# llsurreal919/Reduce-Complexity-for-intra-coding-of-VVC

Hardware: NVIDIA B200
Metric: all-intra 1080p10 CTUs/sec (exhaustive RMD sweep: intra pred + SAD/SATD + mode cost + candidate lists) (higher is better)
Workload: dtype int16 samples / int32 arithmetic / f64 costs

## Files before the change

vvc_intra_b200/csrc/vvcb_api.cu:

```cuda
#include <cuda_runtime.h>
#include <stdio.h>
#include <string.h>
#include <stdlib.h>
#include <math.h>
#include <new>
#include "vvcb_rmd.cuh"
#include "vvcb_tu.cuh"
#include "vvcb_feat.cuh"
#include "vvcb_dq.cuh"
#include "vvcb_rate.cuh"
#include "vvcb_chroma.cuh"
#include <vector>
#include <algorithm>
#include <time.h>
#include <thread>
#include <atomic>
#include "vvcb_romfill.h"

template <int KIND>
__global__ void __launch_bounds__(256) int_peak_kernel(const int* in, int* out, int iters)
{
  int a[8], b[8];
  const int k0 = in[threadIdx.x & 31], k1 = in[32 + (threadIdx.x & 31)];
#pragma unroll
// ... 6 lines not shown
        if (KIND == 0)      { a[i] = a[i] * k1 + k0; b[i] = b[i] * k0 + k1; }
        else if (KIND == 1) { a[i] = (a[i] + k1) ^ k0; b[i] = (b[i] ^ k1) + k0; }
        else                { a[i] = a[i] * k1 + k0; b[i] = (b[i] + k1) ^ k0; }
      }
    }
  }
  int s = 0;
#pragma unroll
  for (int i = 0; i < 8; i++) s += a[i] ^ b[i];
  out[blockIdx.x * blockDim.x + threadIdx.x] = s;
}

constexpr int kSideStreams = 7;
enum Slot {
  kTuIn, kTuOut,
  kTuResi, kTuCoeff,
  kDqCoeff, kDqTabs, kDqScratch, kDqLists,
  kStageIn, kStageOut,
  kOrig, kReco,
  kVisits, kResults, kDetails,
  kBrief,
  kSadSatd,
  kItems,
  kPred,
  kRects, kRectSamples,
  kFeatIn, kFeatOut,
  kChroma,
  kChromaIo,
  kPinTuIn, kPinTuOut, kPinStageIn, kPinStageOut,
  kSlots
};
struct Scratch { void* p; size_t cap; bool pinned; };
struct vvcb_ctx {
  int device, bd, ctu;
  cudaStream_t stream;
  cudaEvent_t ev0, ev1;
  Rom* dRom;
  TrRom* dTrRom;
  Scratch mem[kSlots];
  DqRom* dDqRom;
  RateRom* dRateRom;
  int depQuant;
  float tuMs[4]; int tuTimed; cudaEvent_t tev[5];
  cudaStream_t sIn, sOut; cudaEvent_t evIn[2], evComp[2], evOut[2];
  cudaStream_t sKind[kSideStreams]; cudaEvent_t evPlan, evKind[kSideStreams];
  int evalStreams;
  vvcb_rmd_visit* dVisP[2]; vvcb_rmd_result* dResP[2]; bool pipeReady;
  int trusted;
  const int16_t* bOrig; const int16_t* bReco;
  int width, height, stride;
  PlanState* dPlan;
  int numSms;
  int16_t* wReco;
  int yieldSync; cudaEvent_t evYield;
  void* remote;
  uint64_t launches;
  uint64_t cuNs[8], cuCalls, tuWaitFrom;
  cudaEvent_t cev[4]; bool cuSpan;
  int timing; int timedLaunches; float kms[3]; cudaEvent_t kev[4];
  int cw, ch, cstride;
  char err[512];
};

static char g_createErr[512] = "";

#define CK(call)                                                                                          \
  do {                                                                                                    \
    cudaError_t e_ = (call);                                                                              \
// ... 77 lines not shown
  memset(ctx, 0, sizeof(*ctx));
  ctx->device = device; ctx->bd = bit_depth; ctx->ctu = ctu_size; ctx->depQuant = 1;
  for (int s = kPinTuIn; s < kSlots; s++) ctx->mem[s].pinned = true;
  auto fail = [&](const char* what, cudaError_t err) {
    snprintf(g_createErr, sizeof(g_createErr), "vvcb_create: %s: %s", what, cudaGetErrorString(err));
    vvcb_destroy(ctx);
    return VVCB_ERR_CUDA;
  };
  if ((e = cudaSetDevice(device)) != cudaSuccess) return fail("cudaSetDevice", e);
  cudaDeviceProp prop;
  if ((e = cudaGetDeviceProperties(&prop, device)) != cudaSuccess) return fail("cudaGetDeviceProperties", e);
  ctx->numSms = prop.multiProcessorCount;
  if ((e = cudaStreamCreateWithFlags(&ctx->stream, cudaStreamNonBlocking)) != cudaSuccess) return fail("cudaStreamCreate", e);
  {
    const char* env = getenv("VVCB_EVAL_STREAMS");
    const int v = env ? atoi(env) : 0;
    ctx->evalStreams = v >= 1 && v <= kSideStreams + 1 ? v : kSideStreams + 1;
  }
  for (int i = 0; i < kSideStreams; i++) {
    if ((e = cudaStreamCreateWithFlags(&ctx->sKind[i], cudaStreamNonBlocking)) != cudaSuccess) return fail("cudaStreamCreate", e);
    if ((e = cudaEventCreateWithFlags(&ctx->evKind[i], cudaEventDisableTiming)) != cudaSuccess) return fail("cudaEventCreate", e);
  }
  if ((e = cudaEventCreateWithFlags(&ctx->evPlan, cudaEventDisableTiming)) != cudaSuccess) return fail("cudaEventCreate", e);
  if ((e = cudaEventCreate(&ctx->ev0)) != cudaSuccess) return fail("cudaEventCreate", e);
  if ((e = cudaEventCreateWithFlags(&ctx->evYield, cudaEventBlockingSync | cudaEventDisableTiming)) != cudaSuccess) return fail("cudaEventCreate", e);
  if ((e = cudaEventCreate(&ctx->ev1)) != cudaSuccess) return fail("cudaEventCreate", e);
  for (int i = 0; i < 4; i++) if ((e = cudaEventCreate(&ctx->kev[i])) != cudaSuccess) return fail("cudaEventCreate", e);
  for (int i = 0; i < 4; i++) if ((e = cudaEventCreate(&ctx->cev[i])) != cudaSuccess) return fail("cudaEventCreate", e);
  for (int i = 0; i < 5; i++) if ((e = cudaEventCreate(&ctx->tev[i])) != cudaSuccess) return fail("cudaEventCreate", e);
  Rom* h = new Rom();
  fill_rom(*h);
  if ((e = cudaMalloc(&ctx->dRom, sizeof(Rom))) != cudaSuccess) { delete h; return fail("cudaMalloc(rom)", e); }
  e = cudaMemcpy(ctx->dRom, h, sizeof(Rom), cudaMemcpyHostToDevice);
  delete h;
  if (e != cudaSuccess) return fail("cudaMemcpy(rom)", e);
  if ((e = cudaMalloc(&ctx->dPlan, sizeof(PlanState))) != cudaSuccess) return fail("cudaMalloc(plan)", e);
  {
    TrRom* t = new TrRom();
    fill_tr_rom(*t);
    if ((e = cudaMalloc(&ctx->dTrRom, sizeof(TrRom))) != cudaSuccess) { delete t; return fail("cudaMalloc(trrom)", e); }
    e = cudaMemcpy(ctx->dTrRom, t, sizeof(TrRom), cudaMemcpyHostToDevice);
    delete t;
    if (e != cudaSuccess) return fail("cudaMemcpy(trrom)", e);
  }
  {
    DqRom* t = new DqRom();
// ... 12 lines not shown
  *out = ctx;
  return VVCB_OK;
}

extern "C" void vvcb_destroy(vvcb_ctx* ctx)
{
  if (!ctx) return;
  if (ctx->remote) { vvcbc_disconnect(ctx->remote); delete ctx; return; }
  cudaSetDevice(ctx->device);
  cudaStreamSynchronize(ctx->stream);
  for (Scratch& b : ctx->mem) release(b);
  cudaFree(ctx->dRom); cudaFree(ctx->dPlan); cudaFree(ctx->dTrRom); cudaFree(ctx->dRateRom); cudaFree(ctx->dDqRom);
  if (ctx->pipeReady) {
    cudaStreamSynchronize(ctx->sIn); cudaStreamSynchronize(ctx->sOut);
    for (int i = 0; i < 2; i++) { cudaFree(ctx->dVisP[i]); cudaFree(ctx->dResP[i]); cudaEventDestroy(ctx->evIn[i]); cudaEventDestroy(ctx->evComp[i]); cudaEventDestroy(ctx->evOut[i]); }
    cudaStreamDestroy(ctx->sIn); cudaStreamDestroy(ctx->sOut);
  }
  cudaEventDestroy(ctx->ev0); cudaEventDestroy(ctx->ev1); cudaEventDestroy(ctx->evYield);
  for (int i = 0; i < 4; i++) cudaEventDestroy(ctx->kev[i]);
  for (int i = 0; i < 4; i++) cudaEventDestroy(ctx->cev[i]);
  for (int i = 0; i < 5; i++) cudaEventDestroy(ctx->tev[i]);
  for (int i = 0; i < kSideStreams; i++) { cudaStreamSynchronize(ctx->sKind[i]); cudaStreamDestroy(ctx->sKind[i]); cudaEventDestroy(ctx->evKind[i]); }
  cudaEventDestroy(ctx->evPlan);
  cudaStreamDestroy(ctx->stream);
  delete ctx;
}

extern "C" int vvcb_set_option(vvcb_ctx* ctx, int option, int value)
{
  if (!ctx) return VVCB_ERR_ARG;
  if (option == VVCB_OPT_DEP_QUANT && (value == 0 || value == 1)) {
    ctx->depQuant = value;
    return ctx->remote ? vvcbc_set_option(ctx->remote, option, value, ctx->err, sizeof(ctx->err)) : VVCB_OK;
  }
  if (option == VVCB_OPT_YIELD_SYNC && value >= 0 && value <= 1000) { ctx->yieldSync = value; return VVCB_OK; }
  if (option == VVCB_OPT_TRUSTED_VISITS && (value == 0 || value == 1)) { ctx->trusted = value; return VVCB_OK; }
  snprintf(ctx->err, sizeof(ctx->err), "vvcb_set_option: unknown option %d or bad value %d", option, value);
  return VVCB_ERR_ARG;
}

static int own_planes(vvcb_ctx* ctx, int width, int height)
{
  const int pitch = (width + 63) & ~63;
  const size_t bytes = (size_t)pitch * height * sizeof(int16_t);
  int rc;
  if ((rc = grow(ctx, kOrig, bytes)) || (rc = grow(ctx, kReco, bytes))) return rc;
// ... 187 lines not shown
  }
  ctx->bOrig = static_cast<const int16_t*>(d_orig); ctx->bReco = static_cast<const int16_t*>(d_reco); ctx->wReco = nullptr;
  ctx->width = width; ctx->height = height; ctx->stride = stride;
  return VVCB_OK;
}

extern "C" int vvcb_kernel_timing(vvcb_ctx* ctx, int on)
{
  if (!ctx) return VVCB_ERR_ARG;
  ctx->timing = on; ctx->timedLaunches = 0; ctx->kms[0] = ctx->kms[1] = ctx->kms[2] = 0.f;
  ctx->tuTimed = 0; ctx->tuMs[0] = ctx->tuMs[1] = ctx->tuMs[2] = ctx->tuMs[3] = 0.f;
  return VVCB_OK;
}

extern "C" int vvcb_kernel_times(vvcb_ctx* ctx, float ms[3], int* launches)
{
  if (!ctx || !ms) return VVCB_ERR_ARG;
  for (int i = 0; i < 3; i++) ms[i] = ctx->kms[i];
  if (launches) *launches = ctx->timedLaunches;
  ctx->timedLaunches = 0; ctx->kms[0] = ctx->kms[1] = ctx->kms[2] = 0.f;
  return VVCB_OK;
}

template <int TILE, int KIND, int MODE> static void launch_eval_bucket(const EvalParams& P, int numSms, long long maxWarps, cudaStream_t stream)
{
  using Cfg = EvalCfg<MODE == 1>;
  long long grid = (long long)numSms * Cfg::kMinCtas;
  const long long maxCtas = (maxWarps + Cfg::kWarps - 1) / Cfg::kWarps;
  if (grid > maxCtas) grid = maxCtas;
  if (grid < 1) grid = 1;
  rmd_eval_kernel<TILE, KIND, MODE><<<(int)grid, Cfg::kThreads, 0, stream>>>(P);
}

static int launch_rmd(vvcb_ctx* ctx, const vvcb_rmd_visit* dVisits, int n, vvcb_rmd_result* dResults, vvcb_rmd_detail* dDetails,
                      int16_t* dPred, const vvcb_rmd_visit* hostVisits = nullptr, vvcb_rmd_brief* dBrief = nullptr)
{
  if (!ctx->bOrig) { snprintf(ctx->err, sizeof(ctx->err), "vvcb_rmd_eval: vvcb_frame_begin has not been called"); return VVCB_ERR_STATE; }
  if (n == 0) return VVCB_OK;
  static_assert(kItemTasks >= 128, "the item bound below assumes at least 128 lane-tasks per plain work item");
  int rc;
  if ((rc = grow(ctx, kItems, ((size_t)n * 60 + 8) * sizeof(WorkItem))) || (rc = grow(ctx, kSadSatd, (size_t)n * 2 * VVCB_NUM_SLOTS * sizeof(uint32_t)))) return rc;
  WorkItem* dItems = buf<WorkItem>(ctx, kItems);
  uint32_t* dScratch = buf<uint32_t>(ctx, kSadSatd);
  const bool smallPlan = hostVisits && n <= 4096;
  if (!smallPlan) CK(cudaMemsetAsync(ctx->dPlan, 0, sizeof(PlanState), ctx->stream));
  const bool tm = ctx->timing != 0;
  if (tm) CK(cudaEventRecord(ctx->kev[0], ctx->stream));
  const int pack = dPred ? 0 : 1;
  bool needAll = !hostVisits || n > 4096, need[2][kNumBuckets] = {};
  int inBucket[2][kNumBuckets] = {};
  if (!needAll)
    for (int i = 0; i < n; i++) {
      const vvcb_rmd_visit& v = hostVisits[i];
      const Shape sh = make_shape(v.log2w, v.log2h);
      const int packed = pack && small_shape_index(sh.lw, sh.lh) >= 0 ? 1 : 0;
      const bool mip = !(v.flags & VVCB_VISIT_NO_MIP) && mip_num_modes(sh.w, sh.h) > 0;
      need[packed][sh.tile * kNumKinds + KIND_ANG] = need[packed][sh.tile * kNumKinds + KIND_PDC] = true;
      inBucket[packed][sh.tile * kNumKinds + KIND_ANG]++; inBucket[packed][sh.tile * kNumKinds + KIND_PDC]++;
      if (mip) { need[packed][sh.tile * kNumKinds + KIND_MIP] = true; inBucket[packed][sh.tile * kNumKinds + KIND_MIP]++; }
    }
  int evalLaunches = 0;
  if (smallPlan) rmd_plan_small<<<1, 256, 0, ctx->stream>>>(dVisits, n, ctx->ctu, ctx->dPlan, dItems, pack);
  else {
    rmd_plan_count<<<(n + 255) / 256, 256, 0, ctx->stream>>>(dVisits, n, ctx->ctu, ctx->dPlan, pack);
    rmd_plan_scan<<<1, 32, 0, ctx->stream>>>(ctx->dPlan);
    rmd_plan_fill<<<(n + 255) / 256, 256, 0, ctx->stream>>>(dVisits, n, ctx->ctu, ctx->dPlan, dItems, pack);
  }
  if (tm) CK(cudaEventRecord(ctx->kev[1], ctx->stream));
  EvalParams P;
  P.visits = dVisits; P.items = dItems; P.plan = ctx->dPlan;
  P.sadSM = dScratch; P.satdSM = (dDetails || dPred) ? dScratch + (size_t)VVCB_NUM_SLOTS * n : nullptr; P.nVisits = n;
  P.orig = ctx->bOrig; P.reco = ctx->bReco; P.stride = ctx->stride; P.bd = ctx->bd; P.ctu = ctx->ctu; P.rom = ctx->dRom;
  P.predOut = dPred;
  const long long maxWarps = (long long)n * 8;
  static const int kindOrder[kNumKinds] = { KIND_ANG, KIND_MIP, KIND_PDC };
  static const int tileOrder[kNumClasses] = { 3, 4, 5, 1, 2, 0 };
  if (!needAll && !dPred) {
    for (int mode = 1; mode >= 0; mode--) {
      EvalAny A;
      A.n = 0;
      int cta = 0;
      const int warpsPerCta = mode ? EvalCfg<true>::kWarps : EvalCfg<false>::kWarps, minCtas = mode ? EvalCfg<true>::kMinCtas : EvalCfg<false>::kMinCtas;
      for (int ki = 0; ki < kNumKinds; ki++)
        for (int ti = 0; ti < kNumClasses; ti++) {
          const int b = tileOrder[ti] * kNumKinds + kindOrder[ki];
          if (!need[mode][b] || (mode == 0 && b < kNumKinds)) continue;
          int ctas = (inBucket[mode][b] * 8 + warpsPerCta - 1) / warpsPerCta;
          if (ctas > ctx->numSms * minCtas) ctas = ctx->numSms * minCtas;
          A.bucket[A.n] = (unsigned char)b; A.firstCta[A.n] = cta; cta += ctas; A.n++;
        }
      A.firstCta[A.n] = cta;
      if (!A.n) continue;
      if (mode) rmd_eval_any_kernel<1><<<cta, EvalCfg<true>::kThreads, 0, ctx->stream>>>(P, A);
      else      rmd_eval_any_kernel<0><<<cta, EvalCfg<false>::kThreads, 0, ctx->stream>>>(P, A);
      evalLaunches++;
    }
  } else {
  const int useStreams = needAll ? ctx->evalStreams : (ctx->evalStreams < 3 ? ctx->evalStreams : 3);
  const int nSide = useStreams - 1;
  CK(cudaEventRecord(ctx->evPlan, ctx->stream));
  for (int i = 0; i < nSide; i++) CK(cudaStreamWaitEvent(ctx->sKind[i], ctx->evPlan, 0));
  int dealt = 0;
  auto next_stream = [&]() { const int k = dealt++ % useStreams; return k == 0 ? ctx->stream : ctx->sKind[k - 1]; };
  for (int ki = 0; ki < kNumKinds; ki++)
    for (int ti = 0; ti < kNumClasses; ti++) {
      const int b = tileOrder[ti] * kNumKinds + kindOrder[ki];
      if (dPred) { if (needAll || need[0][b]) { VVCB_FOR_BUCKET(b, 2, launch_eval_bucket, P, ctx->numSms, maxWarps, next_stream()); evalLaunches++; } continue; }
      if (needAll || need[1][b]) { VVCB_FOR_BUCKET(b, 1, launch_eval_bucket, P, ctx->numSms, maxWarps, next_stream()); evalLaunches++; }
      if (b >= kNumKinds && (needAll || need[0][b])) { VVCB_FOR_BUCKET(b, 0, launch_eval_bucket, P, ctx->numSms, maxWarps, next_stream()); evalLaunches++; }
    }
  for (int i = 0; i < nSide; i++) { CK(cudaEventRecord(ctx->evKind[i], ctx->sKind[i])); CK(cudaStreamWaitEvent(ctx->stream, ctx->evKind[i], 0)); }
  }
  if (tm) CK(cudaEventRecord(ctx->kev[2], ctx->stream));
  if (dDetails) { rmd_detail_kernel<<<(n + 31) / 32, 256, 0, ctx->stream>>>(dVisits, n, ctx->ctu, dDetails, P.sadSM, P.satdSM); ctx->launches++; }
  rmd_lists_kernel<<<(n + kListThreads - 1) / kListThreads, kListThreads, 0, ctx->stream>>>(dVisits, n, ctx->ctu, dResults, dDetails, P.sadSM, P.satdSM, dBrief);
  ctx->launches += (smallPlan ? 1 : 3) + evalLaunches + 1;
  CK(cudaGetLastError());
  if (tm) {
    CK(cudaEventRecord(ctx->kev[3], ctx->stream));
    CK(cudaEventSynchronize(ctx->kev[3]));
    for (int i = 0; i < 3; i++) { float ms = 0; CK(cudaEventElapsedTime(&ms, ctx->kev[i], ctx->kev[i + 1])); ctx->kms[i] += ms; }
    ctx->timedLaunches++;
  }
  return VVCB_OK;
}

static bool qp_ok(const vvcb_ctx* ctx, int per, int rem) { return rem >= 0 && rem < 6 && per >= 0 && 6 * per + rem <= 63 + 6 * (ctx->bd - 8); }
static bool lambda_ok(double l) { return l > 0.0 && isfinite(l); }

template <class F> static int first_bad_index(int n, F ok)
{
  const int kMinPerThread = 32768;
  static int maxThreads = 0;
// ... 1594 lines not shown
```

vvc_intra_b200/csrc/vvcb_rmd.cuh:

```cuda
#pragma once
#include "vvcb_core.cuh"

using namespace vvcb;

namespace {

#ifndef VVCB_EVAL_WARPS
#define VVCB_EVAL_WARPS 8
#endif
constexpr int kWarpsPerCta = VVCB_EVAL_WARPS;
constexpr int kThreads     = kWarpsPerCta * 32;
constexpr int KIND_ANG = 0, KIND_PDC = 1, KIND_MIP = 2;

template <int LMAX> struct VisitSmem {
  int16_t lines[kNumSets][2][LMAX];
  int16_t mipBnd[8];
  int16_t mipIn[2][8];
  int     mipAux[4];
  int     pad;
};
using WarpSmem = VisitSmem<kLineMax>;

#ifndef VVCB_PACK_VISITS
#define VVCB_PACK_VISITS 8
#endif
constexpr int kPackVisits  = VVCB_PACK_VISITS;
constexpr int kLineSmall   = 52;
constexpr int kSmallShapes = 8;
constexpr int kNumBucketsAll = kNumBuckets + kSmallShapes * kNumKinds;
static_assert((sizeof(VisitSmem<kLineSmall>) / 4) % 2 == 1, "bank stride of the packed line sets");

__host__ __device__ __forceinline__ int small_shape_index(int lw, int lh)
{
  if (lw + lh > 7 || lw > 4 || lh > 4) return -1;
  if (lw == 2 && lh == 2) return 0;
  if (lw == 3 && lh == 2) return 1;
  if (lw == 2 && lh == 3) return 2;
  if (lw == 3 && lh == 3) return 3;
  if (lw == 4 && lh == 2) return 4;
  if (lw == 2 && lh == 4) return 5;
  if (lw == 4 && lh == 3) return 6;
  return 7;
}

struct PlanState {
  unsigned count[kNumBucketsAll];
  unsigned offset[kNumBucketsAll];
  unsigned fill[kNumBucketsAll];
  unsigned cursor[kNumBucketsAll];
};

#ifndef VVCB_SCRATCH_VISIT_MAJOR
#define VVCB_SCRATCH_VISIT_MAJOR 1
#endif
__host__ __device__ __forceinline__ size_t scratch_at(int slot, unsigned visit, int nVisits)
{
#if VVCB_SCRATCH_VISIT_MAJOR
  (void)nVisits;
  return (size_t)visit * VVCB_NUM_SLOTS + (size_t)slot;
#else
  return (size_t)slot * (size_t)nVisits + visit;
#endif
}

struct EvalParams {
  const vvcb_rmd_visit* visits;
  const WorkItem*       items;
  PlanState*            plan;
  uint32_t*             sadSM;
  uint32_t*             satdSM;
  int                   nVisits;
  const int16_t*        orig;
  const int16_t*        reco;
  int                   stride;
  int                   bd, ctu;
  const Rom*            rom;
  int16_t*              predOut;
};

__device__ __forceinline__ bool visit_mrl_allowed(const vvcb_rmd_visit& v, int ctu)
{
  return !(v.flags & VVCB_VISIT_NO_MRL) && (v.y & (ctu - 1)) != 0;
}

__device__ __forceinline__ int visit_num_mip(const vvcb_rmd_visit& v)
{
  return (v.flags & VVCB_VISIT_NO_MIP) ? 0 : mip_num_modes(1 << v.log2w, 1 << v.log2h);
}

__device__ __forceinline__ int mpm_dc_pos(const vvcb_rmd_visit& v)
{
  int pos = 0;
#pragma unroll
  for (int i = 5; i >= 1; i--) if (v.mpm[i] == 1) pos = i;
  return pos;
}

__device__ __forceinline__ int kind_slot_count(const vvcb_rmd_visit& v, int kind, int ctu)
{
  const bool mrl = visit_mrl_allowed(v, ctu);
// ... 13 lines not shown
  }
  if (idx < 65) return rom.angOrder[v.log2w - 2][v.log2h - 2][idx];
  const int per = 5 - (dc ? 1 : 0);
  const int j = idx - 65;
  const int li = j >= per ? 1 : 0;
  int i = 1 + (j - li * per);
  if (dc && i >= dc) i++;
  return (li ? VVCB_SLOT_MRL3 : VVCB_SLOT_MRL1) + i - 1;
}

__device__ __forceinline__ int items_of(int nSlots, int lanes, int& perItem, bool packed)
{
  if (packed) { perItem = nSlots; return nSlots ? 1 : 0; }
  perItem = lanes >= kItemTasks ? 1 : kItemTasks / lanes;
  return (nSlots + perItem - 1) / perItem;
}

__device__ __forceinline__ int bucket_of(const Shape& sh, int kind, bool packed)
{
  const int small = packed ? small_shape_index(sh.lw, sh.lh) : -1;
  return small >= 0 ? kNumBuckets + small * kNumKinds + kind : sh.tile * kNumKinds + kind;
}

__global__ void rmd_plan_count(const vvcb_rmd_visit* visits, int n, int ctu, PlanState* plan, int pack)
{
  __shared__ unsigned hist[kNumBucketsAll];
  if (threadIdx.x < kNumBucketsAll) hist[threadIdx.x] = 0;
  __syncthreads();
  const int i = blockIdx.x * blockDim.x + threadIdx.x;
  if (i < n) {
    const vvcb_rmd_visit v = visits[i];
    const Shape sh = make_shape(v.log2w, v.log2h);
    const bool packed = pack && small_shape_index(sh.lw, sh.lh) >= 0;
    for (int kind = 0; kind < kNumKinds; kind++) {
      int perItem;
      const int nItems = items_of(kind_slot_count(v, kind, ctu), sh.lanes, perItem, packed);
      if (nItems) atomicAdd(&hist[bucket_of(sh, kind, packed)], (unsigned)nItems);
    }
  }
  __syncthreads();
  if (threadIdx.x < kNumBucketsAll && hist[threadIdx.x]) atomicAdd(&plan->count[threadIdx.x], hist[threadIdx.x]);
}

__global__ void rmd_plan_scan(PlanState* plan)
{
  if (blockIdx.x == 0 && threadIdx.x == 0) {
    unsigned acc = 0;
    for (int b = 0; b < kNumBucketsAll; b++) { plan->offset[b] = acc; acc += plan->count[b]; plan->fill[b] = 0; plan->cursor[b] = 0; }
  }
}

__global__ void rmd_plan_fill(const vvcb_rmd_visit* visits, int n, int ctu, PlanState* plan, WorkItem* items, int pack)
{
  __shared__ unsigned hist[kNumBucketsAll], base[kNumBucketsAll];
  if (threadIdx.x < kNumBucketsAll) hist[threadIdx.x] = 0;
  __syncthreads();
  const int i = blockIdx.x * blockDim.x + threadIdx.x;
  vvcb_rmd_visit v;
  Shape sh = make_shape(2, 2);
  unsigned local[kNumKinds] = { 0, 0, 0 };
  int nItems[kNumKinds] = { 0, 0, 0 }, perItem[kNumKinds] = { 1, 1, 1 }, nSlots[kNumKinds] = { 0, 0, 0 };
  bool packed = false;
  if (i < n) {
    v = visits[i];
    sh = make_shape(v.log2w, v.log2h);
    packed = pack && small_shape_index(sh.lw, sh.lh) >= 0;
    for (int kind = 0; kind < kNumKinds; kind++) {
      nSlots[kind] = kind_slot_count(v, kind, ctu);
      nItems[kind] = items_of(nSlots[kind], sh.lanes, perItem[kind], packed);
      if (nItems[kind]) local[kind] = atomicAdd(&hist[bucket_of(sh, kind, packed)], (unsigned)nItems[kind]);
    }
  }
  __syncthreads();
  if (threadIdx.x < kNumBucketsAll && hist[threadIdx.x])
    base[threadIdx.x] = plan->offset[threadIdx.x] + atomicAdd(&plan->fill[threadIdx.x], hist[threadIdx.x]);
  __syncthreads();
  if (i < n)
    for (int kind = 0; kind < kNumKinds; kind++) {
      const unsigned at = base[bucket_of(sh, kind, packed)] + local[kind];
      for (int k = 0; k < nItems[kind]; k++) {
        WorkItem w;
        w.visit = (uint32_t)i;
        w.slot_begin = (uint16_t)(k * perItem[kind]);
        w.slot_count = (uint16_t)vmin(perItem[kind], nSlots[kind] - k * perItem[kind]);
        items[at + k] = w;
      }
    }
}

__global__ void __launch_bounds__(256) rmd_plan_small(const vvcb_rmd_visit* visits, int n, int ctu, PlanState* plan, WorkItem* items, int pack)
{
  __shared__ unsigned cnt[kNumBucketsAll], off[kNumBucketsAll], cur[kNumBucketsAll];
  for (int b = threadIdx.x; b < kNumBucketsAll; b += blockDim.x) cnt[b] = 0;
  __syncthreads();
  for (int i = threadIdx.x; i < n; i += blockDim.x) {
    const vvcb_rmd_visit v = visits[i];
    const Shape sh = make_shape(v.log2w, v.log2h);
    const bool packed = pack && small_shape_index(sh.lw, sh.lh) >= 0;
    for (int kind = 0; kind < kNumKinds; kind++) {
// ... 99 lines not shown
      for (int u = 0; u < 2; u++) {
        const int i = i0 + 32 * u;
        val[q][u] = i < c[q].total ? load_line_entry(c[q], base, stride, bd, i) : 0;
      }
#pragma unroll
    for (int q = 0; q < NS; q++)
#pragma unroll
      for (int u = 0; u < 2; u++) {
        const int i = i0 + 32 * u;
        if (i < c[q].total) store_line_entry(sm, q ? q + 1 : 0, c[q], i, val[q][u]);
      }
  }
}

template <int UNIT = 4, class SM>
__device__ void build_line_set(SM& sm, int set, int mrl, const vvcb_rmd_visit& v, const Shape& sh,
                               const int16_t* reco, int stride, int bd, int lane)
{
  const LineCtx c = make_line_ctx<UNIT>(v, sh, mrl);
  const int16_t* base = reco + (size_t)v.y * stride + v.x;
  for (int i = lane; i < c.total; i += 32) store_line_entry(sm, set, c, i, load_line_entry(c, base, stride, bd, i));
}

template <class SM>
__device__ void build_filtered_set(SM& sm, const Shape& sh, int lane)
{
  const int nTop = 2 * sh.w + 1, nLeft = 2 * sh.h + 1;
  const int16_t* top = sm.lines[0][0];
  const int16_t* left = sm.lines[0][1];
  for (int i = lane; i < nTop + 2; i += 32) {
    int v;
    if (i == 0) v = (left[1] + 2 * top[0] + top[1] + 2) >> 2;
    else if (i >= nTop - 1) v = top[i];
    else v = (top[i - 1] + 2 * top[i] + top[i + 1] + 2) >> 2;
    sm.lines[1][0][i] = (int16_t)v;
    if (i == 0) sm.lines[1][1][0] = (int16_t)v;
  }
  for (int i = 1 + lane; i < nLeft + 2; i += 32) {
    int v;
    if (i >= nLeft - 1) v = left[i];
    else v = (left[i - 1] + 2 * left[i] + left[i + 1] + 2) >> 2;
    sm.lines[1][1][i] = (int16_t)v;
  }
}

template <class SM>
// ... 247 lines not shown
  static constexpr int kVisits  = PACK ? kPackVisits : 1;
  using Smem = VisitSmem<PACK ? kLineSmall : kLineMax>;
};

__host__ __device__ __forceinline__ int pack_shape_count(int tile) { return tile == 1 || tile == 2 ? 2 : 1; }
__host__ __device__ __forceinline__ int pack_shape(int tile, int i)
{
  return tile == 0 ? 0 : tile == 1 ? (i ? 4 : 1) : tile == 2 ? (i ? 5 : 2) : tile == 3 ? 3 : tile == 4 ? 6 : 7;
}

template <bool PACK> struct EvalShared {
  using Cfg = EvalCfg<PACK>;
  typename Cfg::Smem smem[Cfg::kWarps][Cfg::kVisits];
  int16_t sScratch[Cfg::kWarps][kSlotLineWords];
  vvcb_rmd_visit sVisit[Cfg::kWarps][Cfg::kVisits];
  int sSlots[Cfg::kWarps][Cfg::kVisits + 1];
  unsigned sIndex[Cfg::kWarps][Cfg::kVisits];
  uint32_t sFilt[64];
};

template <int TILE, int KIND, int MODE> constexpr bool kLaneMip = KIND == KIND_MIP && TILE < 4 && MODE != 0;
constexpr int kMipLaneWords = 10 * 34;

template <int TILE, int KIND, int MODE>
__device__ __forceinline__ void rmd_eval_body(const EvalParams& P, EvalShared<MODE == 1>& shm, uint32_t* sMip)
{
  constexpr bool PACK = MODE == 1, WITH_PRED = MODE == 2;
  using Cfg = EvalCfg<PACK>;
  using SM = typename Cfg::Smem;
  constexpr int S = TILE < 3 ? 4 : 8;
  constexpr int V = Cfg::kVisits;
  constexpr bool LANE_MIP = kLaneMip<TILE, KIND, MODE>;
  constexpr bool ONLY_LANE_MIP = LANE_MIP && PACK && (TILE == 0 || TILE == 3);
  constexpr int MIP_FAMILY = TILE == 0 ? 0 : 1;
  auto& smem = shm.smem;
  auto& sScratch = shm.sScratch;
  auto& sVisit = shm.sVisit;
  auto& sSlots = shm.sSlots;
  auto& sIndex = shm.sIndex;
  auto& sFilt = shm.sFilt;
  const int lane = threadIdx.x & 31, warp = threadIdx.x >> 5;
  if (threadIdx.x < 64) sFilt[threadIdx.x] = (&P.rom->filt[0][0])[threadIdx.x];
  if (LANE_MIP)
    for (int i = threadIdx.x; i < mip_family_words(MIP_FAMILY); i += Cfg::kThreads) sMip[i] = P.rom->mip[mip_family_base(MIP_FAMILY) + i];
  __syncthreads();
  const Rom& rom = *P.rom;

#pragma unroll 1
  for (int ps = 0; ps < (PACK ? pack_shape_count(TILE) : 1); ps++) {
  const int BUCKET = PACK ? kNumBuckets + pack_shape(TILE, ps) * kNumKinds + KIND : TILE * kNumKinds + KIND;
  const unsigned nItems = P.plan->count[BUCKET];
  const WorkItem* items = P.items + P.plan->offset[BUCKET];

  for (;;) {
    unsigned it = 0;
    if (lane == 0) it = atomicAdd(&P.plan->cursor[BUCKET], (unsigned)V);
    it = __shfl_sync(0xffffffffu, it, 0);
    if (it >= nItems) break;
    const int nv = PACK ? (int)(nItems - it < (unsigned)V ? nItems - it : (unsigned)V) : 1;
    const WorkItem item = items[it];
    __syncwarp();
#pragma unroll 1
    for (int i = lane; i < nv * 20; i += 32) {
      const int j = i / 20, k = i - j * 20;
      reinterpret_cast<uint32_t*>(&sVisit[warp][j])[k] = reinterpret_cast<const uint32_t*>(P.visits + items[it + j].visit)[k];
    }
    if (lane < nv) sIndex[warp][lane] = items[it + lane].visit;
    __syncwarp();
    const Shape sh = make_shape(sVisit[warp][0].log2w, sVisit[warp][0].log2h);
    const MipGeom mg = make_mip_geom(sh.w, sh.h);
    int maxSlots = PACK ? 0 : (int)item.slot_count;
    if (PACK) {
      int c = lane < nv ? kind_slot_count(sVisit[warp][lane], KIND, P.ctu) : 0;
      if (lane < V) sSlots[warp][lane] = c;
      for (int o = V >> 1; o > 0; o >>= 1) c = vmax(c, __shfl_xor_sync(0xffffffffu, c, o));
      maxSlots = __shfl_sync(0xffffffffu, c, 0);
    }

#pragma unroll 1
    for (int j = 0; j < nv; j++) {
      const vvcb_rmd_visit& v = sVisit[warp][j];
      SM& sm = smem[warp][j];
      int nSets = 1;
      if (KIND != KIND_MIP) {
        const int lastSlot = kind_slot(rom, v, KIND, PACK ? kind_slot_count(v, KIND, P.ctu) - 1 : item.slot_begin + item.slot_count - 1);
        if (lastSlot >= VVCB_SLOT_MRL1) nSets = 3;
      }
      if (KIND == KIND_PDC) {
        if (nSets == 3) build_line_sets<3>(sm, v, sh, P.reco, P.stride, P.bd, lane);
        else            build_line_sets<1>(sm, v, sh, P.reco, P.stride, P.bd, lane);
      } else {
#pragma unroll 1
        for (int q = 0; q < nSets; q++) build_line_set(sm, q ? q + 1 : 0, q == 2 ? 3 : q, v, sh, P.reco, P.stride, P.bd, lane);
      }
    }
    __syncwarp();
#pragma unroll 1
    for (int j = 0; j < nv; j++) {
      if (KIND != KIND_MIP) build_filtered_set(smem[warp][j], sh, lane);
      else                  build_mip_inputs(smem[warp][j], sh, mg, P.bd, lane);
    }
    __syncwarp();

    const int lanes = sh.lanes;
    const int gsize = lanes > 32 ? 32 : lanes;
    const int lgG   = lanes > 32 ? 5 : sh.lgLanes;
    const int gidx  = lane >> lgG, gl = lane & (gsize - 1);
    int16_t* scratch = sScratch[warp] + gidx * ((kSlotLineWords / 32) << lgG);
    const int lgV = !PACK ? 0 : nv > 4 ? 3 : nv > 2 ? 2 : nv > 1 ? 1 : 0;
    const int nTasks = (maxSlots << lgV) * lanes;
    int accSad = 0, accSatd = 0;

    for (int base = 0; base < nTasks; base += 32) {
      const int task = base + lane;
      bool act = task < nTasks;
      int tk = act ? task : nTasks - 1;
      int vi = 0;
      if (PACK) {
        const int r = tk >> sh.lgLanes;
        vi = r & ((1 << lgV) - 1);
        int idx = r >> lgV;
// ... 130 lines not shown
          if (P.satdSM) { P.sadSM[at] = (uint32_t)sad; P.satdSM[at] = (uint32_t)satd; }
          else P.sadSM[at] = (uint32_t)vmin(2 * sad, satd);
        }
      } else {
        accSad += sad; accSatd += satd;
        if (((base >> 5) & 1) == 1) {
          for (int o = 16; o > 0; o >>= 1) {
            accSad  += __shfl_xor_sync(0xffffffffu, accSad, o);
            accSatd += __shfl_xor_sync(0xffffffffu, accSatd, o);
          }
          if (lane == 0) {
            const size_t at = scratch_at(slot, vIdx, P.nVisits);
            if (P.satdSM) { P.sadSM[at] = (uint32_t)accSad; P.satdSM[at] = (uint32_t)accSatd; }
            else P.sadSM[at] = (uint32_t)vmin(2 * accSad, accSatd);
          }
          accSad = 0; accSatd = 0;
        }
      }
    }
  }
  }
}

template <int TILE, int KIND, int MODE>
__global__ void __launch_bounds__(EvalCfg<MODE == 1>::kThreads, EvalCfg<MODE == 1>::kMinCtas) rmd_eval_kernel(EvalParams P)
{
  __shared__ EvalShared<MODE == 1> shm;
  if constexpr (kLaneMip<TILE, KIND, MODE>) {
    alignas(16) __shared__ uint32_t sMip[kMipLaneWords];
    rmd_eval_body<TILE, KIND, MODE>(P, shm, sMip);
  } else rmd_eval_body<TILE, KIND, MODE>(P, shm, nullptr);
}

struct EvalAny {
  int n;
  int firstCta[19];
  unsigned char bucket[20];
};

template <int MODE>
__global__ void __launch_bounds__(EvalCfg<MODE == 1>::kThreads, EvalCfg<MODE == 1>::kMinCtas) rmd_eval_any_kernel(EvalParams P, EvalAny A)
{
  __shared__ EvalShared<MODE == 1> shm;
  alignas(16) __shared__ uint32_t sMip[MODE == 0 ? 1 : kMipLaneWords];
  int k = 0;
  while (k + 1 < A.n && (int)blockIdx.x >= A.firstCta[k + 1]) k++;
  switch (A.bucket[k]) {
    case 0:  rmd_eval_body<0, 0, MODE>(P, shm, sMip); break;  case 1:  rmd_eval_body<0, 1, MODE>(P, shm, sMip); break;  case 2:  rmd_eval_body<0, 2, MODE>(P, shm, sMip); break;
    case 3:  rmd_eval_body<1, 0, MODE>(P, shm, sMip); break;  case 4:  rmd_eval_body<1, 1, MODE>(P, shm, sMip); break;  case 5:  rmd_eval_body<1, 2, MODE>(P, shm, sMip); break;
    case 6:  rmd_eval_body<2, 0, MODE>(P, shm, sMip); break;  case 7:  rmd_eval_body<2, 1, MODE>(P, shm, sMip); break;  case 8:  rmd_eval_body<2, 2, MODE>(P, shm, sMip); break;
    case 9:  rmd_eval_body<3, 0, MODE>(P, shm, sMip); break;  case 10: rmd_eval_body<3, 1, MODE>(P, shm, sMip); break;  case 11: rmd_eval_body<3, 2, MODE>(P, shm, sMip); break;
    case 12: rmd_eval_body<4, 0, MODE>(P, shm, sMip); break;  case 13: rmd_eval_body<4, 1, MODE>(P, shm, sMip); break;  case 14: rmd_eval_body<4, 2, MODE>(P, shm, sMip); break;
    case 15: rmd_eval_body<5, 0, MODE>(P, shm, sMip); break;  case 16: rmd_eval_body<5, 1, MODE>(P, shm, sMip); break;  case 17: rmd_eval_body<5, 2, MODE>(P, shm, sMip); break;
  }
}

struct TuPredParams {
  const vvcb_rmd_visit* visits;
  const vvcb_tu_src*    src;
  const vvcb_tu_job*    jobs;
  int                   n;
  int16_t*              pred;
  int16_t*              resi;
  const int16_t*        orig;
  const int16_t*        reco;
  int                   stride, bd, ctu;
  const Rom*            rom;
};

constexpr int kTuPredWarps = 4;

__global__ void __launch_bounds__(kTuPredWarps * 32) tu_pred_kernel(TuPredParams P)
{
  __shared__ WarpSmem smem[kTuPredWarps];
  __shared__ int16_t sScratch[kTuPredWarps][kSlotLineWords];
  __shared__ uint32_t sFilt[64];
// ... 516 lines not shown
```

Baseline: 14560.

## Stage reference line sets once in PDC kernels and reuse them in ANG/MIP

Adds a per-visit global line-record buffer, with offsets computed during planning and grouped by block shape. The PDC eval kernels build the reference line sets from the reconstructed picture and write them out. The ANG and MIP kernels then copy them back into shared memory instead of rebuilding them. This removes repeated neighbour gathering and padding work across the three mode kinds. In exchange it adds global traffic and extra buffers, and it creates event dependencies between streams that serialise each PDC launch ahead of the ANG/MIP launches for the same tile and mode.

New measurement: 14770 (median of 6 runs). 1.01x the previous value.

```diff
diff --git a/vvc_intra_b200/csrc/vvcb_api.cu b/vvc_intra_b200/csrc/vvcb_api.cu
--- a/vvc_intra_b200/csrc/vvcb_api.cu
+++ b/vvc_intra_b200/csrc/vvcb_api.cu
@@ -52,6 +52,7 @@
   kBrief,
   kSadSatd,
   kItems,
+  kLines, kLineOff,
   kPred,
   kRects, kRectSamples,
   kFeatIn, kFeatOut,
@@ -74,6 +75,7 @@
   float tuMs[4]; int tuTimed; cudaEvent_t tev[5];
   cudaStream_t sIn, sOut; cudaEvent_t evIn[2], evComp[2], evOut[2];
   cudaStream_t sKind[kSideStreams]; cudaEvent_t evPlan, evKind[kSideStreams];
+  cudaEvent_t evStage[2][kNumClasses];
   int evalStreams;
   vvcb_rmd_visit* dVisP[2]; vvcb_rmd_result* dResP[2]; bool pipeReady;
   int trusted;
@@ -197,6 +199,8 @@
     if ((e = cudaEventCreateWithFlags(&ctx->evKind[i], cudaEventDisableTiming)) != cudaSuccess) return fail("cudaEventCreate", e);
   }
   if ((e = cudaEventCreateWithFlags(&ctx->evPlan, cudaEventDisableTiming)) != cudaSuccess) return fail("cudaEventCreate", e);
+  for (auto& ev : ctx->evStage)
+    for (cudaEvent_t& s : ev) if ((e = cudaEventCreateWithFlags(&s, cudaEventDisableTiming)) != cudaSuccess) return fail("cudaEventCreate", e);
   if ((e = cudaEventCreate(&ctx->ev0)) != cudaSuccess) return fail("cudaEventCreate", e);
   if ((e = cudaEventCreateWithFlags(&ctx->evYield, cudaEventBlockingSync | cudaEventDisableTiming)) != cudaSuccess) return fail("cudaEventCreate", e);
   if ((e = cudaEventCreate(&ctx->ev1)) != cudaSuccess) return fail("cudaEventCreate", e);
@@ -255,6 +259,7 @@
   for (int i = 0; i < 5; i++) cudaEventDestroy(ctx->tev[i]);
   for (int i = 0; i < kSideStreams; i++) { cudaStreamSynchronize(ctx->sKind[i]); cudaStreamDestroy(ctx->sKind[i]); cudaEventDestroy(ctx->evKind[i]); }
   cudaEventDestroy(ctx->evPlan);
+  for (auto& ev : ctx->evStage) for (cudaEvent_t s : ev) if (s) cudaEventDestroy(s);
   cudaStreamDestroy(ctx->stream);
   delete ctx;
 }
@@ -488,14 +493,18 @@
   return VVCB_OK;
 }
 
-template <int TILE, int KIND, int MODE> static void launch_eval_bucket(const EvalParams& P, int numSms, long long maxWarps, cudaStream_t stream)
+template <int TILE, int KIND, int MODE, bool STAGED = false> static void launch_eval_bucket(const EvalParams& P, int numSms, long long maxWarps, cudaStream_t stream)
 {
   using Cfg = EvalCfg<MODE == 1>;
   long long grid = (long long)numSms * Cfg::kMinCtas;
   const long long maxCtas = (maxWarps + Cfg::kWarps - 1) / Cfg::kWarps;
   if (grid > maxCtas) grid = maxCtas;
   if (grid < 1) grid = 1;
-  rmd_eval_kernel<TILE, KIND, MODE><<<(int)grid, Cfg::kThreads, 0, stream>>>(P);
+  rmd_eval_kernel<TILE, KIND, MODE, STAGED><<<(int)grid, Cfg::kThreads, 0, stream>>>(P);
+}
+template <int TILE, int KIND, int MODE> static void launch_eval_staged(const EvalParams& P, int numSms, long long maxWarps, cudaStream_t stream)
+{
+  launch_eval_bucket<TILE, KIND, MODE, true>(P, numSms, maxWarps, stream);
 }
 
 static int launch_rmd(vvcb_ctx* ctx, const vvcb_rmd_visit* dVisits, int n, vvcb_rmd_result* dResults, vvcb_rmd_detail* dDetails,
@@ -509,6 +518,13 @@
   WorkItem* dItems = buf<WorkItem>(ctx, kItems);
   uint32_t* dScratch = buf<uint32_t>(ctx, kSadSatd);
   const bool smallPlan = hostVisits && n <= 4096;
+  const bool staged = !smallPlan && !dPred;
+  if (staged) {
+    int recWords = 0;
+    for (int lw = 2; lw <= 6; lw++) for (int lh = 2; lh <= 6; lh++) recWords = std::max(recWords, make_line_record(lw, lh).end[5]);
+    if ((rc = grow(ctx, kLines, (size_t)n * recWords * sizeof(uint32_t))) || (rc = grow(ctx, kLineOff, (size_t)n * sizeof(unsigned long long)))) return rc;
+  }
+  unsigned long long* dLineOff = staged ? buf<unsigned long long>(ctx, kLineOff) : nullptr;
   if (!smallPlan) CK(cudaMemsetAsync(ctx->dPlan, 0, sizeof(PlanState), ctx->stream));
   const bool tm = ctx->timing != 0;
   if (tm) CK(cudaEventRecord(ctx->kev[0], ctx->stream));
@@ -530,7 +546,7 @@
   else {
     rmd_plan_count<<<(n + 255) / 256, 256, 0, ctx->stream>>>(dVisits, n, ctx->ctu, ctx->dPlan, pack);
     rmd_plan_scan<<<1, 32, 0, ctx->stream>>>(ctx->dPlan);
-    rmd_plan_fill<<<(n + 255) / 256, 256, 0, ctx->stream>>>(dVisits, n, ctx->ctu, ctx->dPlan, dItems, pack);
+    rmd_plan_fill<<<(n + 255) / 256, 256, 0, ctx->stream>>>(dVisits, n, ctx->ctu, ctx->dPlan, dItems, pack, dLineOff);
   }
   if (tm) CK(cudaEventRecord(ctx->kev[1], ctx->stream));
   EvalParams P;
@@ -538,6 +554,7 @@
   P.sadSM = dScratch; P.satdSM = (dDetails || dPred) ? dScratch + (size_t)VVCB_NUM_SLOTS * n : nullptr; P.nVisits = n;
   P.orig = ctx->bOrig; P.reco = ctx->bReco; P.stride = ctx->stride; P.bd = ctx->bd; P.ctu = ctx->ctu; P.rom = ctx->dRom;
   P.predOut = dPred;
+  P.lineRec = staged ? buf<uint32_t>(ctx, kLines) : nullptr; P.lineOff = dLineOff;
   const long long maxWarps = (long long)n * 8;
   static const int kindOrder[kNumKinds] = { KIND_ANG, KIND_MIP, KIND_PDC };
   static const int tileOrder[kNumClasses] = { 3, 4, 5, 1, 2, 0 };
@@ -568,13 +585,35 @@
   for (int i = 0; i < nSide; i++) CK(cudaStreamWaitEvent(ctx->sKind[i], ctx->evPlan, 0));
   int dealt = 0;
   auto next_stream = [&]() { const int k = dealt++ % useStreams; return k == 0 ? ctx->stream : ctx->sKind[k - 1]; };
-  for (int ki = 0; ki < kNumKinds; ki++)
-    for (int ti = 0; ti < kNumClasses; ti++) {
-      const int b = tileOrder[ti] * kNumKinds + kindOrder[ki];
-      if (dPred) { if (needAll || need[0][b]) { VVCB_FOR_BUCKET(b, 2, launch_eval_bucket, P, ctx->numSms, maxWarps, next_stream()); evalLaunches++; } continue; }
-      if (needAll || need[1][b]) { VVCB_FOR_BUCKET(b, 1, launch_eval_bucket, P, ctx->numSms, maxWarps, next_stream()); evalLaunches++; }
-      if (b >= kNumKinds && (needAll || need[0][b])) { VVCB_FOR_BUCKET(b, 0, launch_eval_bucket, P, ctx->numSms, maxWarps, next_stream()); evalLaunches++; }
-    }
+  if (dPred) {
+    for (int ki = 0; ki < kNumKinds; ki++)
+      for (int ti = 0; ti < kNumClasses; ti++) {
+        const int b = tileOrder[ti] * kNumKinds + kindOrder[ki];
+        if (needAll || need[0][b]) { VVCB_FOR_BUCKET(b, 2, launch_eval_bucket, P, ctx->numSms, maxWarps, next_stream()); evalLaunches++; }
+      }
+  } else {
+    for (int ti = 0; ti < kNumClasses; ti++)
+      for (int mode = 1; mode >= 0; mode--) {
+        const int t = tileOrder[ti], b = t * kNumKinds + KIND_PDC;
+        if (mode == 0 && t == 0) continue;
+        cudaStream_t s = next_stream();
+        if (mode) { VVCB_FOR_BUCKET(b, 1, launch_eval_staged, P, ctx->numSms, maxWarps, s); }
+        else      { VVCB_FOR_BUCKET(b, 0, launch_eval_staged, P, ctx->numSms, maxWarps, s); }
+        CK(cudaEventRecord(ctx->evStage[mode][t], s));
+        evalLaunches++;
+      }
+    for (int ki = 0; ki < 2; ki++)
+      for (int ti = 0; ti < kNumClasses; ti++)
+        for (int mode = 1; mode >= 0; mode--) {
+          const int t = tileOrder[ti], b = t * kNumKinds + kindOrder[ki];
+          if (mode == 0 && t == 0) continue;
+          cudaStream_t s = next_stream();
+          CK(cudaStreamWaitEvent(s, ctx->evStage[mode][t], 0));
+          if (mode) { VVCB_FOR_BUCKET(b, 1, launch_eval_staged, P, ctx->numSms, maxWarps, s); }
+          else      { VVCB_FOR_BUCKET(b, 0, launch_eval_staged, P, ctx->numSms, maxWarps, s); }
+          evalLaunches++;
+        }
+  }
   for (int i = 0; i < nSide; i++) { CK(cudaEventRecord(ctx->evKind[i], ctx->sKind[i])); CK(cudaStreamWaitEvent(ctx->stream, ctx->evKind[i], 0)); }
   }
   if (tm) CK(cudaEventRecord(ctx->kev[2], ctx->stream));
diff --git a/vvc_intra_b200/csrc/vvcb_rmd.cuh b/vvc_intra_b200/csrc/vvcb_rmd.cuh
--- a/vvc_intra_b200/csrc/vvcb_rmd.cuh
+++ b/vvc_intra_b200/csrc/vvcb_rmd.cuh
@@ -43,11 +43,30 @@
   return 7;
 }
 
+constexpr int kLineShapes = 25;
+struct LineRecord { int end[6]; };
+
+__host__ __device__ __forceinline__ LineRecord make_line_record(int lw, int lh)
+{
+  LineRecord r;
+  int acc = 0;
+#pragma unroll
+  for (int q = 0; q < 3; q++) {
+    const int mrl = q == 2 ? 3 : q;
+    acc += (2 * (1 << lw) + 3 + mrl + (mrl << (lw > lh ? lw - lh : 0)) + 1) >> 1; r.end[2 * q] = acc;
+    acc += (2 * (1 << lh) + 3 + mrl + (mrl << (lh > lw ? lh - lw : 0)) + 1) >> 1; r.end[2 * q + 1] = acc;
+  }
+  return r;
+}
+
 struct PlanState {
   unsigned count[kNumBucketsAll];
   unsigned offset[kNumBucketsAll];
   unsigned fill[kNumBucketsAll];
   unsigned cursor[kNumBucketsAll];
+  unsigned shapeCount[kLineShapes];
+  unsigned shapeFill[kLineShapes];
+  unsigned long long lineBase[kLineShapes];
 };
 
 #ifndef VVCB_SCRATCH_VISIT_MAJOR
@@ -76,6 +95,8 @@
   int                   bd, ctu;
   const Rom*            rom;
   int16_t*              predOut;
+  uint32_t*             lineRec;
+  const unsigned long long* lineOff;
 };
 
 __device__ __forceinline__ bool visit_mrl_allowed(const vvcb_rmd_visit& v, int ctu)
@@ -135,10 +156,13 @@
   return small >= 0 ? kNumBuckets + small * kNumKinds + kind : sh.tile * kNumKinds + kind;
 }
 
+__host__ __device__ __forceinline__ int line_shape(const vvcb_rmd_visit& v) { return (v.log2w - 2) * 5 + v.log2h - 2; }
+
 __global__ void rmd_plan_count(const vvcb_rmd_visit* visits, int n, int ctu, PlanState* plan, int pack)
 {
-  __shared__ unsigned hist[kNumBucketsAll];
+  __shared__ unsigned hist[kNumBucketsAll], shapes[kLineShapes];
   if (threadIdx.x < kNumBucketsAll) hist[threadIdx.x] = 0;
+  if (threadIdx.x < kLineShapes) shapes[threadIdx.x] = 0;
   __syncthreads();
   const int i = blockIdx.x * blockDim.x + threadIdx.x;
   if (i < n) {
@@ -150,9 +174,11 @@
       const int nItems = items_of(kind_slot_count(v, kind, ctu), sh.lanes, perItem, packed);
       if (nItems) atomicAdd(&hist[bucket_of(sh, kind, packed)], (unsigned)nItems);
     }
+    atomicAdd(&shapes[line_shape(v)], 1u);
   }
   __syncthreads();
   if (threadIdx.x < kNumBucketsAll && hist[threadIdx.x]) atomicAdd(&plan->count[threadIdx.x], hist[threadIdx.x]);
+  if (threadIdx.x < kLineShapes && shapes[threadIdx.x]) atomicAdd(&plan->shapeCount[threadIdx.x], shapes[threadIdx.x]);
 }
 
 __global__ void rmd_plan_scan(PlanState* plan)
@@ -160,18 +186,25 @@
   if (blockIdx.x == 0 && threadIdx.x == 0) {
     unsigned acc = 0;
     for (int b = 0; b < kNumBucketsAll; b++) { plan->offset[b] = acc; acc += plan->count[b]; plan->fill[b] = 0; plan->cursor[b] = 0; }
-  }
-}
-
-__global__ void rmd_plan_fill(const vvcb_rmd_visit* visits, int n, int ctu, PlanState* plan, WorkItem* items, int pack)
-{
-  __shared__ unsigned hist[kNumBucketsAll], base[kNumBucketsAll];
+    unsigned long long words = 0;
+    for (int s = 0; s < kLineShapes; s++) {
+      plan->lineBase[s] = words; plan->shapeFill[s] = 0;
+      words += (unsigned long long)plan->shapeCount[s] * make_line_record(2 + s / 5, 2 + s % 5).end[5];
+    }
+  }
+}
+
+__global__ void rmd_plan_fill(const vvcb_rmd_visit* visits, int n, int ctu, PlanState* plan, WorkItem* items, int pack,
+                              unsigned long long* lineOff = nullptr)
+{
+  __shared__ unsigned hist[kNumBucketsAll], base[kNumBucketsAll], shapes[kLineShapes], shapeBase[kLineShapes];
   if (threadIdx.x < kNumBucketsAll) hist[threadIdx.x] = 0;
+  if (threadIdx.x < kLineShapes) shapes[threadIdx.x] = 0;
   __syncthreads();
   const int i = blockIdx.x * blockDim.x + threadIdx.x;
   vvcb_rmd_visit v;
   Shape sh = make_shape(2, 2);
-  unsigned local[kNumKinds] = { 0, 0, 0 };
+  unsigned local[kNumKinds] = { 0, 0, 0 }, rank = 0;
   int nItems[kNumKinds] = { 0, 0, 0 }, perItem[kNumKinds] = { 1, 1, 1 }, nSlots[kNumKinds] = { 0, 0, 0 };
   bool packed = false;
   if (i < n) {
@@ -183,11 +216,17 @@
       nItems[kind] = items_of(nSlots[kind], sh.lanes, perItem[kind], packed);
       if (nItems[kind]) local[kind] = atomicAdd(&hist[bucket_of(sh, kind, packed)], (unsigned)nItems[kind]);
     }
+    if (lineOff) rank = atomicAdd(&shapes[line_shape(v)], 1u);
   }
   __syncthreads();
   if (threadIdx.x < kNumBucketsAll && hist[threadIdx.x])
     base[threadIdx.x] = plan->offset[threadIdx.x] + atomicAdd(&plan->fill[threadIdx.x], hist[threadIdx.x]);
+  if (threadIdx.x < kLineShapes && shapes[threadIdx.x]) shapeBase[threadIdx.x] = atomicAdd(&plan->shapeFill[threadIdx.x], shapes[threadIdx.x]);
   __syncthreads();
+  if (i < n && lineOff) {
+    const int s = line_shape(v);
+    lineOff[i] = plan->lineBase[s] + (unsigned long long)(shapeBase[s] + rank) * make_line_record(sh.lw, sh.lh).end[5];
+  }
   if (i < n)
     for (int kind = 0; kind < kNumKinds; kind++) {
       const unsigned at = base[bucket_of(sh, kind, packed)] + local[kind];
@@ -333,6 +372,36 @@
   for (int i = lane; i < c.total; i += 32) store_line_entry(sm, set, c, i, load_line_entry(c, base, stride, bd, i));
 }
 
+template <bool TO_RECORD, class SM>
+__device__ void copy_line_record(SM& sm, uint32_t* rec, const Shape& sh, int nSets, int lane)
+{
+  constexpr int kLineWords = (int)sizeof(sm.lines[0][0]) / 4;
+  static_assert(sizeof(sm.lines[0][0]) % sizeof(uint32_t) == 0, "line arrays of whole words");
+  const LineRecord r = make_line_record(sh.lw, sh.lh);
+  const int words = nSets == 3 ? r.end[5] : r.end[1];
+  uint32_t* lines = reinterpret_cast<uint32_t*>(&sm.lines[0][0][0]);
+#pragma unroll 1
+  for (int i0 = lane; i0 < words; i0 += 64) {
+    uint32_t val[2];
+    int at[2];
+#pragma unroll
+    for (int u = 0; u < 2; u++) {
+      const int i = i0 + 32 * u;
+      int seg = 0, start = 0;
+#pragma unroll
+      for (int k = 0; k < 5; k++) if (i >= r.end[k]) { seg = k + 1; start = r.end[k]; }
+      const int set = seg >> 1 ? (seg >> 1) + 1 : 0;
+      at[u] = (2 * set + (seg & 1)) * kLineWords + i - start;
+      val[u] = i < words ? (TO_RECORD ? lines[at[u]] : rec[i]) : 0u;
+    }
+#pragma unroll
+    for (int u = 0; u < 2; u++) {
+      const int i = i0 + 32 * u;
+      if (i < words) { if (TO_RECORD) rec[i] = val[u]; else lines[at[u]] = val[u]; }
+    }
+  }
+}
+
 template <class SM>
 __device__ void build_filtered_set(SM& sm, const Shape& sh, int lane)
 {
@@ -626,7 +695,7 @@
 template <int TILE, int KIND, int MODE> constexpr bool kLaneMip = KIND == KIND_MIP && TILE < 4 && MODE != 0;
 constexpr int kMipLaneWords = 10 * 34;
 
-template <int TILE, int KIND, int MODE>
+template <int TILE, int KIND, int MODE, bool STAGED>
 __device__ __forceinline__ void rmd_eval_body(const EvalParams& P, EvalShared<MODE == 1>& shm, uint32_t* sMip)
 {
   constexpr bool PACK = MODE == 1, WITH_PRED = MODE == 2;
@@ -669,7 +738,12 @@
       const int j = i / 20, k = i - j * 20;
       reinterpret_cast<uint32_t*>(&sVisit[warp][j])[k] = reinterpret_cast<const uint32_t*>(P.visits + items[it + j].visit)[k];
     }
-    if (lane < nv) sIndex[warp][lane] = items[it + lane].visit;
+    unsigned long long lineOff = 0;
+    if (lane < nv) {
+      const unsigned vi = items[it + lane].visit;
+      sIndex[warp][lane] = vi;
+      if (STAGED && KIND != KIND_PDC) lineOff = P.lineOff[vi];
+    }
     __syncwarp();
     const Shape sh = make_shape(sVisit[warp][0].log2w, sVisit[warp][0].log2h);
     const MipGeom mg = make_mip_geom(sh.w, sh.h);
@@ -691,8 +765,12 @@
         if (lastSlot >= VVCB_SLOT_MRL1) nSets = 3;
       }
       if (KIND == KIND_PDC) {
-        if (nSets == 3) build_line_sets<3>(sm, v, sh, P.reco, P.stride, P.bd, lane);
-        else            build_line_sets<1>(sm, v, sh, P.reco, P.stride, P.bd, lane);
+        if (nSets == 3 || (STAGED && visit_mrl_allowed(v, P.ctu))) build_line_sets<3>(sm, v, sh, P.reco, P.stride, P.bd, lane);
+        else                                                      build_line_sets<1>(sm, v, sh, P.reco, P.stride, P.bd, lane);
+      } else if (STAGED) {
+        const unsigned long long off = (unsigned long long)__shfl_sync(0xffffffffu, (unsigned)(lineOff >> 32), j) << 32 |
+                                       __shfl_sync(0xffffffffu, (unsigned)lineOff, j);
+        copy_line_record<false>(sm, P.lineRec + off, sh, nSets, lane);
       } else {
 #pragma unroll 1
         for (int q = 0; q < nSets; q++) build_line_set(sm, q ? q + 1 : 0, q == 2 ? 3 : q, v, sh, P.reco, P.stride, P.bd, lane);
@@ -701,6 +779,8 @@
     __syncwarp();
 #pragma unroll 1
     for (int j = 0; j < nv; j++) {
+      if (STAGED && KIND == KIND_PDC)
+        copy_line_record<true>(smem[warp][j], P.lineRec + P.lineOff[sIndex[warp][j]], sh, visit_mrl_allowed(sVisit[warp][j], P.ctu) ? 3 : 1, lane);
       if (KIND != KIND_MIP) build_filtered_set(smem[warp][j], sh, lane);
       else                  build_mip_inputs(smem[warp][j], sh, mg, P.bd, lane);
     }
@@ -877,14 +957,15 @@
   }
 }
 
-template <int TILE, int KIND, int MODE>
+template <int TILE, int KIND, int MODE, bool STAGED = false>
 __global__ void __launch_bounds__(EvalCfg<MODE == 1>::kThreads, EvalCfg<MODE == 1>::kMinCtas) rmd_eval_kernel(EvalParams P)
 {
+  static_assert(!STAGED || MODE != 2, "the prediction-output kernels walk the lines");
   __shared__ EvalShared<MODE == 1> shm;
   if constexpr (kLaneMip<TILE, KIND, MODE>) {
     alignas(16) __shared__ uint32_t sMip[kMipLaneWords];
-    rmd_eval_body<TILE, KIND, MODE>(P, shm, sMip);
-  } else rmd_eval_body<TILE, KIND, MODE>(P, shm, nullptr);
+    rmd_eval_body<TILE, KIND, MODE, STAGED>(P, shm, sMip);
+  } else rmd_eval_body<TILE, KIND, MODE, STAGED>(P, shm, nullptr);
 }
 
 struct EvalAny {
@@ -901,12 +982,12 @@
   int k = 0;
   while (k + 1 < A.n && (int)blockIdx.x >= A.firstCta[k + 1]) k++;
   switch (A.bucket[k]) {
-    case 0:  rmd_eval_body<0, 0, MODE>(P, shm, sMip); break;  case 1:  rmd_eval_body<0, 1, MODE>(P, shm, sMip); break;  case 2:  rmd_eval_body<0, 2, MODE>(P, shm, sMip); break;
-    case 3:  rmd_eval_body<1, 0, MODE>(P, shm, sMip); break;  case 4:  rmd_eval_body<1, 1, MODE>(P, shm, sMip); break;  case 5:  rmd_eval_body<1, 2, MODE>(P, shm, sMip); break;
-    case 6:  rmd_eval_body<2, 0, MODE>(P, shm, sMip); break;  case 7:  rmd_eval_body<2, 1, MODE>(P, shm, sMip); break;  case 8:  rmd_eval_body<2, 2, MODE>(P, shm, sMip); break;
-    case 9:  rmd_eval_body<3, 0, MODE>(P, shm, sMip); break;  case 10: rmd_eval_body<3, 1, MODE>(P, shm, sMip); break;  case 11: rmd_eval_body<3, 2, MODE>(P, shm, sMip); break;
-    case 12: rmd_eval_body<4, 0, MODE>(P, shm, sMip); break;  case 13: rmd_eval_body<4, 1, MODE>(P, shm, sMip); break;  case 14: rmd_eval_body<4, 2, MODE>(P, shm, sMip); break;
-    case 15: rmd_eval_body<5, 0, MODE>(P, shm, sMip); break;  case 16: rmd_eval_body<5, 1, MODE>(P, shm, sMip); break;  case 17: rmd_eval_body<5, 2, MODE>(P, shm, sMip); break;
+    case 0:  rmd_eval_body<0, 0, MODE, false>(P, shm, sMip); break;  case 1:  rmd_eval_body<0, 1, MODE, false>(P, shm, sMip); break;  case 2:  rmd_eval_body<0, 2, MODE, false>(P, shm, sMip); break;
+    case 3:  rmd_eval_body<1, 0, MODE, false>(P, shm, sMip); break;  case 4:  rmd_eval_body<1, 1, MODE, false>(P, shm, sMip); break;  case 5:  rmd_eval_body<1, 2, MODE, false>(P, shm, sMip); break;
+    case 6:  rmd_eval_body<2, 0, MODE, false>(P, shm, sMip); break;  case 7:  rmd_eval_body<2, 1, MODE, false>(P, shm, sMip); break;  case 8:  rmd_eval_body<2, 2, MODE, false>(P, shm, sMip); break;
+    case 9:  rmd_eval_body<3, 0, MODE, false>(P, shm, sMip); break;  case 10: rmd_eval_body<3, 1, MODE, false>(P, shm, sMip); break;  case 11: rmd_eval_body<3, 2, MODE, false>(P, shm, sMip); break;
+    case 12: rmd_eval_body<4, 0, MODE, false>(P, shm, sMip); break;  case 13: rmd_eval_body<4, 1, MODE, false>(P, shm, sMip); break;  case 14: rmd_eval_body<4, 2, MODE, false>(P, shm, sMip); break;
+    case 15: rmd_eval_body<5, 0, MODE, false>(P, shm, sMip); break;  case 16: rmd_eval_body<5, 1, MODE, false>(P, shm, sMip); break;  case 17: rmd_eval_body<5, 2, MODE, false>(P, shm, sMip); break;
   }
 }
 
```
